# pkusys/Auncel

Hardware: AMD Instinct MI355X
Metric: queries/sec @ recall@10>=0.95, SIFT-10M d=128 IVF4096, 1/2/4/8 GPU (higher is better)
Workload: dtype u8

## Files before the change

auncel_amd/csrc/ivf_select.hip:

```cpp
#include "ivf_dev.h"

#include <algorithm>
#include <stdexcept>
#include <stdlib.h>
#include <string.h>
#include <string>
#include <type_traits>
#include <utility>

namespace amdivf {

struct RegHeap {
    uint32_t v0, v1;
    uint32_t s0, s1;
};

__device__ __forceinline__ void wl_u(uint32_t& reg, uint32_t val, int l) {
    uint32_t m0s;
    asm("s_mov_b32 %[m], m0\n\ts_mov_b32 m0, %[l]\n\ts_nop 0\n\tv_writelane_b32 %[r], %[v], m0\n\ts_mov_b32 m0, %[m]"
        : [r] "+v"(reg), [m] "=&s"(m0s)
        : [v] "s"(val), [l] "s"(l));
}

__device__ __forceinline__ void wl2_u(uint32_t& r0, uint32_t v0, uint32_t& r1, uint32_t v1, int l) {
// ... 382 lines not shown
        else high = middle - 1;
    }
    return (uint32_t)(low + 1);
}

constexpr uint32_t CURNUM_PAR_MAXK = 10;
template <bool IsMax>
__device__ inline uint32_t cur_num_par(const TraceLds& tr, const float* lut, const float* srt, const float* dwin, float* terms,
                                       uint32_t query_topk, int lane, uint32_t* err) {
    const int nterm = (int)query_topk * 15;
    unsigned long long errm = 0;
    for (int base = 0; base < nterm; base += 64) {
        const int idx = base + lane;
        uint32_t e = 0;
        if (idx < nterm) {
            const int m = idx / 15, i = idx - m * 15;
            uint32_t e0 = 0;
            const float kd = IsMax ? srt[m] : arcos_lut(lut, srt[m], &e0);
            const float b = dwin[i];
            float t = 0.f;
            if (!(b >= kd)) t = arcos_lut(lut, b / kd, &e);
            terms[idx] = t;
        }
        unsigned long long eb = __ballot(e != 0);
        while (eb) {
            const int l = __builtin_ctzll(eb);
            eb &= eb - 1;
            errm |= 1ull << ((base + l) / 15);
        }
    }
    wave_sync();
    float g = 0.f;
    if ((uint32_t)lane < query_topk) {
        float sum = 0.f;
#pragma unroll
        for (int i = 0; i < 15; i++) sum += terms[lane * 15 + i];
        g = trace_search(tr.x, tr.z, tr.n, sum);
    }
    const unsigned long long query_k = query_topk;
    const bool first_ok = (double)((float)query_k * g) <= (double)query_k * 1.005;
    const bool step_ok = (float)(lane + 1) * g <= (float)query_k;
    const unsigned long long mfirst = __ballot((uint32_t)lane == query_topk - 1 && first_ok);
    const unsigned long long mstep = __ballot((uint32_t)lane < query_topk && step_ok);
    wave_sync();
    unsigned long long high = query_k - 1, low = 0, middle = 0;
    if ((errm >> high) & 1) {
        *err = ERR_ARCOS_DOMAIN;
        return 0;
    }
    if (mfirst) return (uint32_t)query_k;
    while (low <= high) {
        middle = (low + high) / 2;
        if (middle <= 0) return 0;
        if ((errm >> middle) & 1) {
            *err = ERR_ARCOS_DOMAIN;
            return 0;
        }
        if ((mstep >> middle) & 1) low = middle + 1;
        else high = middle - 1;
    }
    return (uint32_t)(low + 1);
}

constexpr uint32_t SKEY_SENT = 0xff7fffffu;
constexpr uint32_t SPOS_NONE = 0xffffffffu;

struct SortedRegs {
    uint32_t k0, k1;
    uint32_t g0, g1;
};

__device__ __forceinline__ uint32_t wave_shr1(uint32_t x, uint32_t carry) {
    return (uint32_t)__builtin_amdgcn_update_dpp((int)carry, (int)x, 0x138 , 0xf, 0xf, false);
}

template <bool TWO> __device__ __forceinline__ uint32_t sr_key(const SortedRegs& r, int i) {
    if (!TWO) return rl_u(r.k0, i);
    const uint32_t a = rl_u(r.k0, i >> 1), b = rl_u(r.k1, i >> 1);
    return (i & 1) ? b : a;
}
template <bool TWO> __device__ __forceinline__ int sr_e0(int lane) { return TWO ? 2 * lane : lane; }
template <bool TWO> __device__ __forceinline__ int sr_e1(int lane) { return TWO ? 2 * lane + 1 : 128; }

template <bool TWO> __device__ __forceinline__ int sr_insert(SortedRegs& r, uint32_t key, uint32_t gpos, int lane) {
    (void)lane;
    const bool w0 = r.k0 > key;
    if (TWO) {
        const bool w1 = r.k1 > key;
        const int at = 128 - __builtin_popcountll(__ballot(w0)) - __builtin_popcountll(__ballot(w1));
        const uint32_t t0 = wave_shr1(r.k1, 0u), u0 = wave_shr1(r.g1, 0u);
        const bool p0 = t0 > key;
        const uint32_t n1k = w0 ? r.k0 : key, n1g = w0 ? r.g0 : gpos;
        r.k1 = w1 ? n1k : r.k1;
        r.g1 = w1 ? n1g : r.g1;
        r.k0 = w0 ? (p0 ? t0 : key) : r.k0;
        r.g0 = w0 ? (p0 ? u0 : gpos) : r.g0;
        return at;
    }
    const int at = 64 - __builtin_popcountll(__ballot(w0));
    const uint32_t t0 = wave_shr1(r.k0, 0u), u0 = wave_shr1(r.g0, 0u);
    const bool p0 = t0 > key;
    r.k0 = w0 ? (p0 ? t0 : key) : r.k0;
    r.g0 = w0 ? (p0 ? u0 : gpos) : r.g0;
    return at;
}

__device__ inline int64_t pair_of_gpos(const uint64_t* list_off, uint32_t nlist, uint32_t gpos) {
    uint32_t lo = 0, hi = nlist;
    while (hi - lo > 1) {
        const uint32_t mid = (lo + hi) >> 1;
        if (list_off[mid] <= gpos) lo = mid;
        else hi = mid;
    }
    return ((int64_t)lo << 32) | (int64_t)(gpos - list_off[lo]);
}

__host__ __device__ inline size_t replay_wave_bytes(int k, uint32_t nlist, bool geo, bool tune, bool train, uint32_t trace_cap) {
    (void)nlist;
    size_t b = (size_t)k * 16;
    if (geo) b += 16 * 4 + 16 * 4;
    if (tune) b += (size_t)trace_cap * 8;
    if (tune) b += CURNUM_PAR_MAXK * 15 * 4 + 8;
    if (train) b += (size_t)k * 4;
    return (b + 15) & ~(size_t)15;
}

template <bool IsMax, bool RH, int NLD, int KC>
__global__ __launch_bounds__(256) __attribute__((amdgpu_waves_per_eu(NLD == 16 ? 5 : 3))) void replay_kernel(ReplayArgs a) {
    extern __shared__ __align__(16) unsigned char smem[];
    const int lane = threadIdx.x & 63;
    const int wave = __builtin_amdgcn_readfirstlane(threadIdx.x >> 6);
    const bool tune = a.tuner.enabled != 0, training = a.train.enabled != 0, geo = tune || training;
    const int k = KC ? KC : a.k;
    const uint32_t nlist = a.nlist;
    const uint32_t max_num = nlist / 8 + 20;

    float* lut = reinterpret_cast<float*>(smem);
    if (geo) {
        const float* g = tune ? a.tuner.arcos : a.train.arcos;
        for (int i = threadIdx.x; i < 500; i += 256) lut[i] = g[i];
        __syncthreads();
    }
    const uint32_t li = blockIdx.x * 4 + wave;
    if (li >= (a.nq_dev ? *a.nq_dev : a.nq)) return;
    const uint32_t qi = a.qsel ? a.qsel[li] : li;
    if (a.done[qi]) return;

    unsigned char* base = smem + (geo ? 2000 : 0) + (size_t)wave * replay_wave_bytes(k, nlist, geo, tune, training, a.trace_cap);
    int64_t* href = reinterpret_cast<int64_t*>(base);
    float* hval = reinterpret_cast<float*>(base + (size_t)k * 8);
    float* srt = hval + k;
    float* dwin = srt + k;
    float* pend = dwin + (geo ? 16 : 0);
    float* trc = pend + (geo ? 16 : 0);
    float* terms = trc + (tune ? 2 * a.trace_cap : 0);
    float* gtrow = terms + (tune ? CURNUM_PAR_MAXK * 15 + 2 : 0);
    const float* gdtb = geo ? a.dtb + (size_t)qi * max_num : nullptr;

    for (int i = lane; i < k; i += 64) {
        hval[i] = a.heap_val[(size_t)qi * k + i];
        href[i] = a.heap_ref[(size_t)qi * k + i];
    }
    wave_sync();

    const unsigned long long id_q = a.id_offset + qi;
    const unsigned long long dbg_t0 = a.dbg ? __builtin_readcyclecounter() : 0;
    unsigned long long dbg_evals = 0, dbg_stream = 0, dbg_rule = 0, dbg_chunks = 0, dbg_probes = 0;
    uint32_t err = 0;
    uint32_t ik0 = a.stage[qi];
    const uint32_t loop_end = a.limit ? a.limit[qi] : a.total_nprobe;
    const uint32_t si = a.seg_by_slot ? qi : li;
    const uint32_t cnt = a.seg_count[si];
    const size_t seg0 = a.seg_begin ? (size_t)a.seg_begin[si] : (size_t)li * a.round_probes;
    unsigned long long nscan = a.nscan[qi];
    float pre_val = a.pre_val ? a.pre_val[qi] : 0.f;
    uint32_t stoped = a.stoped ? a.stoped[qi] : 0u;
    unsigned long long st_nlist = 0, st_nheap = 0, st_ndis = 0;

    constexpr bool VTWO = KC == 0 || KC > 63;
    auto stored = [](float x) { return IsMax ? fkey(x) : ~fkey(x); };
    auto unstored = [](uint32_t sk) { return fkey_inv(IsMax ? sk : ~sk); };
    VHeap vh{0u, 0u, 0u, 0u};
    const VHeapLane vc = vh_lane(lane);
    unsigned long long chain0 = 0, chain1 = 0;
    if (RH) {
        if (lane >= 1 && lane <= k) vh.k0 = stored(hval[lane - 1]);
        if (VTWO && lane + 64 <= k) vh.k1 = stored(hval[lane + 63]);
// ... 467 lines not shown
    const unsigned long long lt = (1ull << lane) - 1ull;
    for (uint32_t s0 = (blockIdx.x * 4u + (threadIdx.x >> 6)) * 8u; s0 < nseg; s0 += stride) {
        uint32_t m_n = 0;
        unsigned long long m_off = 0;
        if (lane < 8 && s0 + lane < nseg) {
            const int key = a.seg_list[s0 + lane];
            m_off = a.seg_off[s0 + lane];
            if (key >= 0 && (uint32_t)key < a.nlist) m_n = (uint32_t)(a.list_off[key + 1] - a.list_off[key]);
        }
        unsigned long long W[8];
#pragma unroll
        for (int r = 0; r < 8; r++) {
            const uint32_t n = rl_u(m_n, r);
            const unsigned long long off = ((unsigned long long)rl_u((uint32_t)(m_off >> 32), r) << 32) | rl_u((uint32_t)m_off, r);
            W[r] = (uint32_t)lane < ((n + 63u) >> 6) ? __builtin_nontemporal_load(a.mask + (off >> 6) + lane) : 0ull;
        }
#pragma unroll
        for (int r = 0; r < 8; r++) {
            if (s0 + r >= nseg) break;
            const uint32_t n = rl_u(m_n, r);
            const unsigned long long off = ((unsigned long long)rl_u((uint32_t)(m_off >> 32), r) << 32) | rl_u((uint32_t)m_off, r);
            const unsigned long long* mw = a.mask + (off >> 6) + lane;
            const float* row = a.dist + off + lane;
            const uint32_t words = (n + 63u) >> 6;
            uint32_t total = wave_sum_u32((uint32_t)__builtin_popcountll(W[r]));
            for (uint32_t b = 64; b < words; b += 64u)
                total += wave_sum_u32(b + lane < words ? (uint32_t)__builtin_popcountll(__builtin_nontemporal_load(mw + b)) : 0u);
            total = (uint32_t)__builtin_amdgcn_readfirstlane((int)total);
            uint2* ent = a.cl_ent + (size_t)(s0 + r) * CL_CAP;
            uint32_t report = total;
            if (total > CL_CAP) {
                uint32_t start = a.arena_per_xcd;
                if (lane == 0 && total <= a.arena_per_xcd &&
                    __hip_atomic_load(&a.cursor[32u * xcc_id()], __ATOMIC_RELAXED, __HIP_MEMORY_SCOPE_WORKGROUP) < a.arena_per_xcd)
                    start = xcd_local_add(&a.cursor[32u * xcc_id()], total);
                start = (uint32_t)__builtin_amdgcn_readfirstlane((int)start);
                if (start >= a.arena_per_xcd || total > a.arena_per_xcd - start) {
                    if (lane == 0) a.cl_cnt[s0 + r] = CL_WALK;
                    continue;
                }
                start += xcc_id() * a.arena_per_xcd;
                if (lane == 0) ent[0] = make_uint2(start, 0u);
                ent = a.arena + start;
            }
            uint32_t count = 0;
            auto put = [&](unsigned long long w, uint32_t b, int c, float x) {
                const unsigned long long bits = ((unsigned long long)rl_u((uint32_t)(w >> 32), c) << 32) | rl_u((uint32_t)w, c);
                const bool mine = (bits >> lane) & 1ull;
                const unsigned long long bal = __ballot(mine);
                if (mine) ent[count + (uint32_t)__builtin_popcountll(bal & lt)] = make_uint2((b + (uint32_t)c) * 64u + (uint32_t)lane, __float_as_uint(x));
                count += (uint32_t)__builtin_popcountll(bal);
            };
            for (uint32_t b = 0; b < words; b += 64u) {
                const unsigned long long w = b == 0 ? W[r] : (b + lane < words ? __builtin_nontemporal_load(mw + b) : 0ull);
                unsigned long long nz = __ballot(w != 0ull);
                while (nz) {
                    int c[4] = {-1, -1, -1, -1};
                    float x[4] = {0.f, 0.f, 0.f, 0.f};
#pragma unroll
                    for (int u = 0; u < 4; u++) {
                        if (nz) {
                            c[u] = __builtin_ctzll(nz);
                            nz &= nz - 1;
                            x[u] = __builtin_nontemporal_load(row + (size_t)(b + c[u]) * 64);
                        }
                    }
#pragma unroll
                    for (int u = 0; u < 4; u++)
                        if (c[u] >= 0) put(w, b, c[u], x[u]);
                }
            }
            if (lane == 0) a.cl_cnt[s0 + r] = report;
        }
    }
}

void launch_compact_rows(const CompactArgs& a, hipStream_t s) {
    const uint32_t want = a.nseg_dev ? a.nseg_hint : a.nseg;
    if (want == 0) return;
    const uint32_t grid = std::min<uint32_t>((want + 31u) / 32u, 8192u);
    LAUNCH(compact_rows_kernel, dim3(grid), dim3(256), 0, s, a);
}

template <bool IsMax, bool MASKED, bool TUNE, int KC>
__global__ __launch_bounds__(256) __attribute__((amdgpu_waves_per_eu(MASKED ? 4 : AUNCEL_SEL_WAVES))) void select_sorted_kernel(ReplayArgs a) {
    extern __shared__ __align__(16) unsigned char smem[];
    constexpr bool TWO = KC == 0 || KC > 64;
    const int lane = threadIdx.x & 63;
    const int wave = __builtin_amdgcn_readfirstlane(threadIdx.x >> 6);
    const int k = KC ? KC : a.k;
    const uint32_t nlist = a.nlist;
    const uint32_t max_num = nlist / 8 + 20;
    float* lut = reinterpret_cast<float*>(smem);
    if (TUNE) {
        for (int i = threadIdx.x; i < 500; i += 256) lut[i] = a.tuner.arcos[i];
        __syncthreads();
    }
    const uint32_t li = blockIdx.x * 4 + wave;
    if (li >= (a.nq_dev ? *a.nq_dev : a.nq)) return;
    const uint32_t qi = (uint32_t)__builtin_amdgcn_readfirstlane((int)(a.qsel ? a.qsel[li] : li));
    if (a.done[qi]) return;

    unsigned char* wbase = smem + (TUNE ? 2000 : 0) + (size_t)wave * select_wave_bytes(k, TUNE, !MASKED, a.trace_cap);
    uint32_t* mk = reinterpret_cast<uint32_t*>(wbase);
    uint32_t* mg = mk + 128;
    float* srt = reinterpret_cast<float*>(wbase + SEL_MERGE_BYTES);
    float* dwin = srt + k;
    float* trc = dwin + 16;
    float* terms = trc + (!MASKED && 2 * a.trace_cap < 640u ? 640u : 2 * a.trace_cap);
    uint32_t* fill = reinterpret_cast<uint32_t*>(TUNE ? reinterpret_cast<unsigned char*>(trc) : wbase + SEL_MERGE_BYTES);
    const float* gdtb = TUNE ? a.dtb + (size_t)qi * max_num : nullptr;

    SortedRegs sr{0xffffffffu, 0xffffffffu, SPOS_NONE, SPOS_NONE};
    const int e0 = sr_e0<TWO>(lane), e1 = sr_e1<TWO>(lane);
    if (e0 < k) {
        sr.k0 = okey<IsMax>(a.heap_val[(size_t)qi * k + e0]);
        sr.g0 = (uint32_t)a.heap_ref[(size_t)qi * k + e0];
    }
    if (TWO && e1 < k) {
        sr.k1 = okey<IsMax>(a.heap_val[(size_t)qi * k + e1]);
        sr.g1 = (uint32_t)a.heap_ref[(size_t)qi * k + e1];
    }
    uint32_t amb = (uint32_t)__builtin_amdgcn_readfirstlane((int)a.amb[qi]);
    uint32_t logn = (uint32_t)__builtin_amdgcn_readfirstlane((int)a.log_cnt[qi]);
    uint2* const qlog = a.log + (size_t)qi * a.log_cap;
    uint32_t log_v = 0, log_g = 0;
    if (!AUNCEL_SEL_BATCH && (uint32_t)lane < (logn & 63u)) {
        const uint2 e = qlog[(logn & ~63u) + lane];
        log_v = e.x;
        log_g = e.y;
    }
    auto worst_key = [&]() { return sr_key<TWO>(sr, k - 1); };
    uint32_t topk = worst_key();
    float top = okey_inv<IsMax>(topk);
    auto srt_from_regs = [&]() {
        if (e0 < k) srt[e0] = okey_inv<IsMax>(sr.k0);
        if (TWO && e1 < k) srt[e1] = okey_inv<IsMax>(sr.k1);
    };
    if (TUNE) {
        srt_from_regs();
        wave_sync();
    }

    const unsigned long long id_q = a.id_offset + qi;
    uint32_t err = 0;
    const uint32_t ik0 = (uint32_t)__builtin_amdgcn_readfirstlane((int)a.stage[qi]);
    const uint32_t loop_end = a.limit ? a.limit[qi] : a.total_nprobe;
    const uint32_t cnt = (uint32_t)__builtin_amdgcn_readfirstlane((int)a.seg_count[qi]);
    const size_t seg0 = (size_t)a.seg_begin[qi];
    unsigned long long nscan = a.nscan[qi];
    float pre_val = a.pre_val[qi];
    uint32_t stoped = a.stoped[qi];
    unsigned long long st_nlist = 0, st_ndis = 0;
    uint32_t st_nheap = 0;
    const unsigned long long dbg_t0 = a.dbg ? __builtin_readcyclecounter() : 0;
    unsigned long long dbg_rule = 0;
    uint32_t dbg_evals = 0, dbg_chunks = 0, dbg_walked = 0;

    uint32_t query_k = 0;
    float true_KD_K = 0.f, racc = 0.f;
    unsigned long long np = 0;
    int cached_ind = -1;
    bool have_pre = false, top_changed = true, srt_changed = true;
    uint32_t kept_pre = 0;
    TraceLds tr{trc, trc + a.trace_cap, 0};
    if (TUNE) {
        query_k = a.tuner.query_topk;
        if (a.tuner.gt_D) true_KD_K = a.tuner.gt_D[id_q * (unsigned long long)k + query_k - 1];
        racc = a.tuner.require_acc[id_q];
        np = a.tuner.my_nprobe[id_q];
    }
    const unsigned long long np_in = np;
    const uint32_t nl8 = nlist / 8;
    const bool overhead = TUNE && a.tuner.overhead != 0;
    const float mult = TUNE ? a.tuner.multipler : 1.f;
    const unsigned long long stops = (unsigned long long)(racc * 12);
    float kept_recall = 0.f;

    int ins_min = 128;
#if AUNCEL_SEL_BATCH
    uint32_t B_k = 0, B_g = 0;
    uint32_t bn = 0;
    auto flush = [&]() {
        if (bn == 0) return;
        const bool cand = (uint32_t)lane < bn;
        const uint32_t myk = cand ? B_k : 0xffffffffu;
        uint32_t pa = 0, w = 0, later = 0, sh0 = 0, sh1 = 0;
        for (uint32_t i = 0; i < bn; i++) {
            const uint32_t ki = rl_u(B_k, (int)i);
            uint32_t p = (uint32_t)__builtin_popcountll(__ballot(sr.k0 <= ki));
            if (TWO) p += (uint32_t)__builtin_popcountll(__ballot(sr.k1 <= ki));
            wl_u(pa, (uint32_t)__builtin_amdgcn_readfirstlane((int)p), __builtin_amdgcn_readfirstlane((int)i));
            w += (ki <= myk && (uint32_t)lane > i) ? 1u : 0u;
            later += (ki < myk && (uint32_t)lane < i) ? 1u : 0u;
            sh0 += ki < sr.k0 ? 1u : 0u;
            if (TWO) sh1 += ki < sr.k1 ? 1u : 0u;
        }
        const bool adm = cand && pa + w < (uint32_t)k;
        const unsigned long long am = __ballot(adm);
        const uint32_t nadm = (uint32_t)__builtin_popcountll(am);
        if (nadm) {
            const uint32_t rank = pa + w + later;
            const uint32_t r0 = (uint32_t)e0 + sh0, r1 = (uint32_t)e1 + sh1;
            wave_sync();
            if (e0 < k && r0 < (uint32_t)k) {
                mk[r0] = sr.k0;
                mg[r0] = sr.g0;
            }
            if (TWO && e1 < k && r1 < (uint32_t)k) {
                mk[r1] = sr.k1;
                mg[r1] = sr.g1;
            }
            if (adm && rank < (uint32_t)k) {
                mk[rank] = B_k;
                mg[rank] = B_g;
            }
            if (logn + nadm > a.log_cap) {
                err = ERR_LOG_OVERFLOW;
            } else if (adm) {
                const uint32_t at = logn + (uint32_t)__builtin_popcountll(am & ((1ull << lane) - 1ull));
                qlog[at] = make_uint2(__float_as_uint(okey_inv<IsMax>(B_k)), B_g);
            }
            logn += logn + nadm > a.log_cap ? 0u : nadm;
            st_nheap += nadm;
            const unsigned long long top_in = __ballot(adm && rank < query_k);
            if (top_in) ins_min = 0;
            wave_sync();
            const bool l0 = e0 < k, l1 = TWO && e1 < k;
            const uint32_t wk = mk[k - 1];
            const bool out0 = l0 && r0 >= (uint32_t)k && sr.k0 == wk, out1 = l1 && r1 >= (uint32_t)k && sr.k1 == wk;
            const bool outc = adm && rank >= (uint32_t)k && B_k == wk;
            if (l0) {
                sr.k0 = mk[e0];
                sr.g0 = mg[e0];
            }
            if (l1) {
                sr.k1 = mk[e1];
                sr.g1 = mg[e1];
            }
            if (wk != SKEY_SENT && __ballot(out0 || out1 || outc) != 0) amb = wk;
            topk = wk;
            top = okey_inv<IsMax>(wk);
        }
        bn = 0;
    };
    auto admit = [&](float val, uint32_t ckey, uint32_t gp) {
        (void)val;
        gp = (uint32_t)__builtin_amdgcn_readfirstlane((int)gp);
        wl2_u(B_k, (uint32_t)__builtin_amdgcn_readfirstlane((int)ckey), B_g, gp, __builtin_amdgcn_readfirstlane((int)bn));
        bn++;
        if (bn == 64u) flush();
    };
#else
    auto flush = [&]() {};
    auto admit = [&](float val, uint32_t ckey, uint32_t gp) {
        const uint32_t evicted = topk;
        gp = (uint32_t)__builtin_amdgcn_readfirstlane((int)gp);
        const int at = sr_insert<TWO>(sr, ckey, gp, lane);
        ins_min = at < ins_min ? at : ins_min;
        const uint32_t ln = (uint32_t)__builtin_amdgcn_readfirstlane((int)logn);
        if (ln >= a.log_cap) {
            err = ERR_LOG_OVERFLOW;
        } else {
            const bool me = (uint32_t)lane == (ln & 63u);
            log_v = me ? __float_as_uint(val) : log_v;
            log_g = me ? gp : log_g;
            if ((ln & 63u) == 63u) qlog[(ln & ~63u) + lane] = make_uint2(log_v, log_g);
            logn = ln + 1;
        }
        st_nheap++;
        const uint32_t wk = worst_key();
        if (wk == evicted && wk != SKEY_SENT) amb = wk;
        topk = wk;
        top = okey_inv<IsMax>(wk);
    };
#endif

    uint32_t win0 = 0;
    int m_key = -1;
    uint32_t m_n = 0, m_base = 0;
    const bool lists = MASKED && a.cl_cnt != nullptr;
    uint32_t m_cc = 0;
    uint2 E[8];
    auto load_window = [&](uint32_t w0) {
        win0 = w0;
        m_key = -1;
        m_n = 0;
        m_base = 0;
        const uint32_t pi = w0 + lane;
        if (lists) {
            m_cc = pi < cnt ? a.cl_cnt[seg0 + pi] : 0u;
            const uint2* ep = a.cl_ent + (seg0 + w0) * CL_CAP + lane;
#pragma unroll
            for (int j = 0; j < 8; j++) E[j] = w0 + 8u * j + ((uint32_t)lane >> 3) < cnt ? ep[64 * j] : make_uint2(0u, 0u);
        }
        if (pi < cnt) {
            m_key = a.seg_list[seg0 + pi];
            if (m_key >= 0 && (uint32_t)m_key < nlist) {
                const uint64_t o0 = a.list_off[m_key], o1 = a.list_off[m_key + 1];
                m_n = (uint32_t)(o1 - o0);
                m_base = a.identity_ids ? 0u : (uint32_t)o0;
            }
        }
    };
    load_window(0);
    unsigned long long region_off = cnt ? a.seg_off[seg0] : 0ull;
    region_off = ((unsigned long long)(uint32_t)__builtin_amdgcn_readfirstlane((int)(region_off >> 32)) << 32) |
                 (uint32_t)__builtin_amdgcn_readfirstlane((int)(uint32_t)region_off);

    const float* regionf = a.dist + region_off + lane;
    auto load_block = [&](const float* p) {
        f4 r;
        r.x = __builtin_nontemporal_load(p);
        r.y = __builtin_nontemporal_load(p + 64);
        r.z = __builtin_nontemporal_load(p + 128);
        r.w = __builtin_nontemporal_load(p + 192);
        return r;
    };
    f4 R0, R1, R2, R3;
    uint32_t gpos = 0;
    const unsigned long long* rmask = MASKED ? a.mask + (region_off >> 6) + lane : nullptr;
    const float* region1 = a.dist + region_off + lane;
    unsigned long long W = 0, Wn = 0;
    uint32_t wstep = 0;
    if (!MASKED) {
        R0 = load_block(regionf);
        R1 = load_block(regionf + 256);
        R2 = load_block(regionf + 512);
        R3 = load_block(regionf + 768);
    } else if (!lists) {
        W = __builtin_nontemporal_load(rmask);
        Wn = __builtin_nontemporal_load(rmask + 64);
    }
    uint32_t wpos = 0;

    auto dense_block = [&](const f4 x, uint32_t c0, uint32_t n, uint32_t lbase, uint32_t taken) {
        const uint32_t valid = n > c0 ? n - c0 : 0u;
        const uint32_t skip = taken > c0 ? taken - c0 : 0u;
        const uint32_t p0 = (uint32_t)lane, p1 = 64u + lane, p2 = 128u + lane, p3 = 192u + lane;
        const unsigned long long h0 = __ballot(hcmp<IsMax>(top, x.x) && p0 < valid && p0 >= skip);
        const unsigned long long h1 = __ballot(hcmp<IsMax>(top, x.y) && p1 < valid && p1 >= skip);
        const unsigned long long h2 = __ballot(hcmp<IsMax>(top, x.z) && p2 < valid && p2 >= skip);
        const unsigned long long h3 = __ballot(hcmp<IsMax>(top, x.w) && p3 < valid && p3 >= skip);
        auto walk = [&](unsigned long long h, const float xc, uint32_t g0) {
            while (h) {
                const int l = __builtin_ctzll(h);
                h &= h - 1;
                const float val = rl_f(xc, l);
                const uint32_t ck = okey<IsMax>(val);
                if (ck < topk) admit(val, ck, g0 + (uint32_t)l);
            }
        };
        const uint32_t g0 = lbase + c0;
        walk(h0, x.x, g0);
        walk(h1, x.y, g0 + 64u);
        walk(h2, x.z, g0 + 128u);
        walk(h3, x.w, g0 + 192u);
    };

    auto fill_first_k = [&](const f4 x, uint32_t n, uint32_t lbase) -> uint32_t {
        const uint32_t m = n < (uint32_t)k ? n : (uint32_t)k;
        uint32_t *fk = fill, *fv = fill + 128, *fg = fill + 256, *sk = fill + 384, *sg = fill + 512;
        const float xs[4] = {x.x, x.y, x.z, x.w};
        bool bad = false;
#pragma unroll
        for (int c = 0; c < 4; c++) bad = bad || (64u * c + lane < m && okey<IsMax>(xs[c]) >= SKEY_SENT);
        if (__ballot(bad) != 0) return 0u;
#pragma unroll
        for (int c = 0; c < 4; c++) {
            const uint32_t j = 64u * c + lane;
            if (j < m) {
                fk[j] = okey<IsMax>(xs[c]);
                fv[j] = __float_as_uint(xs[c]);
                fg[j] = lbase + j;
                qlog[j] = make_uint2(__float_as_uint(xs[c]), lbase + j);
            }
        }
        wave_sync();
        const uint32_t j0 = lane, j1 = lane + 64;
        const uint32_t k0v = j0 < m ? fk[j0] : 0u, k1v = j1 < m ? fk[j1] : 0u;
        uint32_t r0 = 0, r1 = 0;
        for (uint32_t i = 0; i < m; i++) {
            const uint32_t ki = fk[i];
            r0 += (ki < k0v || (ki == k0v && i < j0)) ? 1u : 0u;
            r1 += (ki < k1v || (ki == k1v && i < j1)) ? 1u : 0u;
        }
        if (j0 < m) {
            sk[r0] = k0v;
            sg[r0] = fg[j0];
        }
        if (j1 < m) {
            sk[r1] = k1v;
            sg[r1] = fg[j1];
        }
        wave_sync();
        if ((uint32_t)e0 < m) {
            sr.k0 = sk[e0];
            sr.g0 = sg[e0];
        }
        if (TWO && (uint32_t)e1 < m) {
            sr.k1 = sk[e1];
            sr.g1 = sg[e1];
        }
        logn = m;
        if ((uint32_t)lane < (m & 63u)) {
            log_v = fv[(m & ~63u) + lane];
            log_g = fg[(m & ~63u) + lane];
        }
        st_nheap += m;
        ins_min = 0;
        topk = worst_key();
        top = okey_inv<IsMax>(topk);
        wave_sync();
        return m;
    };
    bool fresh = !MASKED && logn == 0 && sr_key<TWO>(sr, 0) == SKEY_SENT;

    bool finished = false;
    uint32_t consumed = 0;
    for (uint32_t p = 0; p < cnt && !finished; p++) {
        const uint32_t ik = ik0 + p;
        consumed = p + 1;
        if (p >= win0 + 64) load_window(p);
        const int key = rl_i(m_key, (int)(p - win0));
        ins_min = 128;
        const uint32_t nheap0 = st_nheap;
        if (key >= 0) {
            if ((uint32_t)key >= nlist) {
                err = ERR_INVALID_KEY;
                finished = true;
                break;
            }
            const uint32_t n = rl_u(m_n, (int)(p - win0));
            if (n > 0) {
                st_nlist++;
                const uint32_t lbase = rl_u(m_base, (int)(p - win0));
                if (!MASKED) {
                    const uint32_t ngrp = (n + 1023u) >> 10;
                    uint32_t taken = 0;
                    if (fresh) {
                        taken = fill_first_k(R0, n, lbase);
                        fresh = false;
                    }
                    for (uint32_t g = 0; g < ngrp; g++) {
                        const float* nxt = regionf + (size_t)(gpos + 1) * 1024;
#define SEL_BLOCK(R, U)                                                                                                       \
    {                                                                                                                         \
        const f4 x = R;                                                                                                       \
        R = load_block(nxt + (U) * 256);                                                                                      \
        const float best = IsMax ? fminf(fminf(fminf(x.x, x.y), x.z), x.w) : fmaxf(fmaxf(fmaxf(x.x, x.y), x.z), x.w);         \
        if (__ballot(hcmp<IsMax>(top, best)) != 0) dense_block(x, g * 1024u + (U) * 256u, n, lbase, taken);                   \
    }
                        SEL_BLOCK(R0, 0)
                        SEL_BLOCK(R1, 1)
                        SEL_BLOCK(R2, 2)
                        SEL_BLOCK(R3, 3)
#undef SEL_BLOCK
                        gpos++;
                    }
                } else {
                    const uint32_t row_w0 = wpos, wend = wpos + ((n + 63u) >> 6);
                    if (lists) {
                        const int r = (int)(p - win0);
                        const uint32_t cc = rl_u(m_cc, r);
                        if (cc <= CL_CAP) {
                            if (cc) {
                                uint2 e = E[0];
#pragma unroll
                                for (int j = 1; j < 8; j++)
                                    if ((r >> 3) == j) e = E[j];
                                const int l0 = (r & 7) * 8;
                                for (uint32_t t = 0; t < cc; t++) {
                                    const float val = __uint_as_float(rl_u(e.y, l0 + (int)t));
                                    const uint32_t ck = okey<IsMax>(val);
                                    if (hcmp<IsMax>(top, val) && ck < topk) admit(val, ck, lbase + rl_u(e.x, l0 + (int)t));
                                }
                            }
                            wpos = wend;
                        } else if (cc != CL_WALK) {
                            uint2 e = E[0];
#pragma unroll
                            for (int j = 1; j < 8; j++)
                                if ((r >> 3) == j) e = E[j];
                            const uint2* al = a.cl_arena + rl_u(e.x, (r & 7) * 8) + lane;
                            for (uint32_t t0 = 0; t0 < cc; t0 += 64u) {
                                const bool in = t0 + (uint32_t)lane < cc;
                                const uint2 o = in ? al[t0] : make_uint2(0u, 0u);
                                unsigned long long m = __ballot(in && hcmp<IsMax>(top, __uint_as_float(o.y)));
                                while (m) {
                                    const int l = __builtin_ctzll(m);
                                    m &= m - 1;
                                    const float val = __uint_as_float(rl_u(o.y, l));
                                    const uint32_t ck = okey<IsMax>(val);
                                    if (ck < topk) admit(val, ck, lbase + rl_u(o.x, l));
                                }
                            }
                            wpos = wend;
                        } else {
                            if (a.dbg) dbg_walked++;
                            wstep = wpos >> 6;
                            W = __builtin_nontemporal_load(rmask + (size_t)wstep * 64);
                            Wn = __builtin_nontemporal_load(rmask + (size_t)(wstep + 1) * 64);
                        }
                    }
                    while (wpos < wend) {
                        const uint32_t s0 = wstep * 64u;
                        if (wpos >= s0 + 64u) {
                            W = Wn;
                            wstep++;
                            Wn = __builtin_nontemporal_load(rmask + (size_t)(wstep + 1) * 64);
                            continue;
                        }
                        const uint32_t lo = wpos - s0, hi = wend - s0 < 64u ? wend - s0 : 64u;
                        unsigned long long nz = __ballot(W != 0ull);
                        nz &= ~0ull << lo;
                        if (hi < 64u) nz &= (1ull << hi) - 1ull;
                        wpos = s0 + hi;
                        while (nz) {
                            int c0 = -1, c1 = -1, c2 = -1, c3 = -1;
                            float x0 = 0.f, x1 = 0.f, x2 = 0.f, x3 = 0.f;
                            c0 = __builtin_ctzll(nz);
                            nz &= nz - 1;
                            x0 = __builtin_nontemporal_load(region1 + (size_t)(s0 + c0) * 64);
                            if (nz) {
                                c1 = __builtin_ctzll(nz);
                                nz &= nz - 1;
                                x1 = __builtin_nontemporal_load(region1 + (size_t)(s0 + c1) * 64);
                            }
                            if (nz) {
                                c2 = __builtin_ctzll(nz);
                                nz &= nz - 1;
                                x2 = __builtin_nontemporal_load(region1 + (size_t)(s0 + c2) * 64);
                            }
                            if (nz) {
                                c3 = __builtin_ctzll(nz);
                                nz &= nz - 1;
                                x3 = __builtin_nontemporal_load(region1 + (size_t)(s0 + c3) * 64);
                            }
                            auto chunk = [&](int c, float x) {
                                if (c < 0) return;
                                if (a.dbg) dbg_chunks++;
                                const unsigned long long bits = ((unsigned long long)rl_u((uint32_t)(W >> 32), c) << 32) | rl_u((uint32_t)W, c);
                                const uint32_t cb = (s0 + (uint32_t)c - row_w0) * 64u;
                                unsigned long long m = __ballot(((bits >> lane) & 1) && hcmp<IsMax>(top, x));
                                while (m) {
                                    const int l = __builtin_ctzll(m);
                                    m &= m - 1;
                                    const float val = rl_f(x, l);
                                    const uint32_t ck = okey<IsMax>(val);
                                    if (ck < topk) admit(val, ck, lbase + cb + (uint32_t)l);
                                }
                            };
                            chunk(c0, x0);
                            chunk(c1, x1);
                            chunk(c2, x2);
                            chunk(c3, x3);
                        }
                    }
                    wpos = row_w0 + (((n + 1023u) >> 10) << 4);
                }
                nscan += n;
                st_ndis += n;
            }
        }
        flush();
        if (TUNE && st_nheap != nheap0) {
            wave_sync();
            srt_from_regs();
            wave_sync();
            srt_changed = true;
            if (ins_min < (int)query_k) top_changed = true;
        }
        if (a.max_codes && nscan >= a.max_codes) {
            finished = true;
            break;
        }
        if (loop_end && ik + 1 >= loop_end) finished = true;
        if (TUNE) {
            const unsigned long long dbg_r0 = a.dbg ? __builtin_readcyclecounter() : 0;
            const uint32_t stage = ik + 1;
            const bool fired = IsMax && np != 0 && !overhead;
            if (!fired) {
                const uint32_t tmp_stage = stage >= nl8 ? nl8 - 1 : stage;
                const uint32_t ind = tmp_stage <= 1u ? 0u : 32u - (uint32_t)__builtin_clz(tmp_stage - 1u);
                if ((int)ind != cached_ind) {
                    const uint32_t o = a.tuner.trace_off[ind], tn = a.tuner.trace_off[ind + 1] - o;
                    const float sc = a.tuner.std_m;
                    wave_sync();
                    for (uint32_t i = lane; i < tn; i += 64) {
                        trc[i] = a.tuner.trace_x[o + i];
                        trc[a.trace_cap + i] = a.tuner.trace_y[o + i] + sc * a.tuner.trace_std[o + i];
                    }
                    if (lane < 15) dwin[lane] = gdtb[(1u << ind) - 1 + lane];
                    tr.n = tn;
                    cached_ind = (int)ind;
                    have_pre = false;
                    wave_sync();
                }
                if (!IsMax && srt_changed) {
                    for (int i = lane; i < k; i += 64) (void)arcos_lut(lut, srt[i], &err);
                    err = wave_err(err);
                    if (err) {
                        finished = true;
                        break;
                    }
                }
                srt_changed = false;
                if (!have_pre || top_changed) {
                    dbg_evals++;
                    kept_pre = query_k <= CURNUM_PAR_MAXK ? cur_num_par<IsMax>(tr, lut, srt, dwin, terms, query_k, lane, &err)
                                                          : cur_num_lds<IsMax>(tr, lut, srt, dwin, query_k, lane, &err);
                    have_pre = true;
                    top_changed = false;
                    err = wave_err(err);
                    if (err) finished = true;
                    kept_recall = (float)kept_pre / (float)query_k;
                }
                float recall = kept_recall;
                const float max_val = IsMax ? fmaxf(-1.f, top) : fminf(FLT_MAX, top);
                if (stage > 1) {
                    if (max_val == pre_val) stoped++;
                    else stoped = 0;
                    if (stoped >= stops) recall = 1;
                }
                pre_val = max_val;
                if (!overhead) {
                    if (recall >= racc && np == 0) {
                        np = (unsigned long long)((float)stage * mult);
                        if (np >= nlist && lane == 0) a.tuner.t_recalls[id_q] = 1.f;
                    }
                    if (stage >= nl8 && np == 0) {
                        np = (unsigned long long)((float)stage * mult);
                        if (np >= nlist && lane == 0) a.tuner.t_recalls[id_q] = 1.f;
                    }
                }
            }
            if (overhead) {
                if (stage >= nl8) finished = true;
            } else if (np != 0 && np <= stage) {
                if (a.tuner.profile) {
                    uint32_t hits = 0;
                    for (int i = lane; i < k; i += 64) {
                        const float s = srt[i];
                        if (IsMax ? ((double)s <= (double)true_KD_K * 1.0005) : ((double)s >= (double)true_KD_K * 0.9995)) hits++;
                    }
                    for (int off = 32; off; off >>= 1) hits += __shfl_xor(hits, off);
                    if (lane == 0) a.tuner.t_recalls[id_q] = (float)hits / (float)query_k;
                }
                finished = true;
            }
            if (a.dbg) dbg_rule += __builtin_readcyclecounter() - dbg_r0;
        }
    }
    err = wave_err(err);

    if (lane == 0) {
        a.stage[qi] = ik0 + consumed;
        a.nscan[qi] = nscan;
        a.pre_val[qi] = pre_val;
        a.stoped[qi] = stoped;
        if (TUNE && np != np_in) a.tuner.my_nprobe[id_q] = np;
        if (a.qstat) {
            uint2 qs = a.qstat[qi];
            qs.x += (uint32_t)st_nlist;
            qs.y += (uint32_t)st_nheap;
            a.qstat[qi] = qs;
        }
        {
            unsigned long long* st = a.stats + 4 * xcc_id();
            if (st_nlist) xcd_local_add64(&st[0], st_nlist);
            if (st_ndis) xcd_local_add64(&st[1], st_ndis);
            if (st_nheap) xcd_local_add64(&st[2], (unsigned long long)st_nheap);
        }
        if (err) atomicMax(a.error, err);
        if (a.dbg) {
            a.dbg[(size_t)li * 8 + 0] = __builtin_readcyclecounter() - dbg_t0;
            a.dbg[(size_t)li * 8 + 1] = st_nheap;
            a.dbg[(size_t)li * 8 + 2] = st_ndis;
            a.dbg[(size_t)li * 8 + 3] = dbg_evals;
            a.dbg[(size_t)li * 8 + 4] = dbg_walked;
            a.dbg[(size_t)li * 8 + 5] = dbg_rule;
            a.dbg[(size_t)li * 8 + 6] = dbg_chunks;
            a.dbg[(size_t)li * 8 + 7] = consumed;
        }
        if (a.thr) a.thr[qi] = top;
        a.log_cnt[qi] = logn;
        a.log_snap[(size_t)(a.round & 1u) * a.nq_total + qi] = logn;
        if (finished || a.finalize_all || err) a.fin_round[qi] = a.round;
    }
    if (!AUNCEL_SEL_BATCH && (uint32_t)lane < (logn & 63u)) qlog[(logn & ~63u) + lane] = make_uint2(log_v, log_g);
    const bool in0 = e0 < k, in1 = TWO && e1 < k;
    if (finished || a.finalize_all || err) {
        const uint32_t p0 = wave_shr1(TWO ? sr.k1 : sr.k0, 0xfffffffeu), p1 = sr.k0;
        const bool dup = (in0 && lane >= 1 && sr.k0 == p0 && sr.k0 != SKEY_SENT) || (in1 && sr.k1 == p1 && sr.k1 != SKEY_SENT);
        const bool tainted = __ballot(dup) != 0 || worst_key() == amb;
        if (tainted && !err) {
            if (lane == 0) {
                a.tie_flag[qi] = 1;
                xcd_local_add64(&a.stats[4 * xcc_id() + 3], 1ull);
            }
        } else {
            auto put = [&](int i, uint32_t key, uint32_t g) {
                const bool empty = key == SKEY_SENT && g == SPOS_NONE;
                int64_t id = -1;
                if (!empty) id = a.identity_ids ? (int64_t)g : a.store_pairs ? pair_of_gpos(a.list_off, nlist, g) : a.ids[g];
                a.D[(size_t)qi * k + i] = empty ? hneutral<IsMax>() : okey_inv<IsMax>(key);
                a.I[(size_t)qi * k + i] = id;
            };
            if (in0) put(e0, sr.k0, sr.g0);
            if (in1) put(e1, sr.k1, sr.g1);
        }
        if (lane == 0) a.done[qi] = 1;
    } else {
        if (in0) {
            a.heap_val[(size_t)qi * k + e0] = okey_inv<IsMax>(sr.k0);
            a.heap_ref[(size_t)qi * k + e0] = sr.g0 == SPOS_NONE ? -1 : (int64_t)sr.g0;
        }
        if (in1) {
            a.heap_val[(size_t)qi * k + e1] = okey_inv<IsMax>(sr.k1);
            a.heap_ref[(size_t)qi * k + e1] = sr.g1 == SPOS_NONE ? -1 : (int64_t)sr.g1;
        }
        if (lane == 0) {
            a.amb[qi] = amb;
            if (a.unfinished) (void)xcd_local_add(&a.unfinished[xcc_id()], 1u);
        }
    }
}

void launch_select_sorted(const ReplayArgs& a, hipStream_t s) {
    if (a.nq == 0) return;
    const bool tune = a.tuner.enabled != 0;
    const size_t shmem = (tune ? 2000 : 0) + 4 * select_wave_bytes(a.k, tune, a.mask == nullptr, a.trace_cap);
    if (shmem > 160 * 1024) throw std::runtime_error("selection kernel: trace cache beyond LDS");
    const dim3 grid((a.nq + 3) / 4), block(256);
    auto go = [&](auto kern) {
        const hipError_t e = hipFuncSetAttribute(reinterpret_cast<const void*>(kern), hipFuncAttributeMaxDynamicSharedMemorySize, (int)shmem);
        if (e != hipSuccess) throw std::runtime_error(std::string("selection kernel: cannot reserve LDS: ") + hipGetErrorString(e));
        LAUNCH(kern, grid, block, shmem, s, a);
    };
    auto pick_k = [&](auto is_max, auto masked, auto tn) {
        constexpr bool M = decltype(is_max)::value, MK = decltype(masked)::value, T = decltype(tn)::value;
        if (a.k == 100) return go(select_sorted_kernel<M, MK, T, 100>);
        if (a.k == 10) return go(select_sorted_kernel<M, MK, T, 10>);
        return go(select_sorted_kernel<M, MK, T, 0>);
    };
    auto pick_t = [&](auto is_max, auto masked) {
        if (tune) pick_k(is_max, masked, std::true_type{});
        else pick_k(is_max, masked, std::false_type{});
    };
    auto pick_m = [&](auto is_max) {
        if (a.mask) pick_t(is_max, std::true_type{});
        else pick_t(is_max, std::false_type{});
    };
    if (a.metric == METRIC_L2) pick_m(std::true_type{});
    else pick_m(std::false_type{});
}

bool replay_sorted_applies(const ReplayArgs& a) {
    return a.log != nullptr && a.k >= 1 && a.k <= 128 && !a.train.enabled && !a.raw_heap_out;
}

void launch_replay(const ReplayArgs& a, hipStream_t s) {
    if (a.nq == 0) return;
    const bool tune = a.tuner.enabled != 0, train = a.train.enabled != 0, geo = tune || train;
    const size_t shmem = (geo ? 2000 : 0) + 4 * replay_wave_bytes(a.k, a.nlist, geo, tune, train, a.trace_cap);
    const dim3 grid((a.nq + 3) / 4), block(256);
    static const bool no_rh = getenv("AUNCEL_AMD_LDS_HEAP") != nullptr;
    if (replay_sorted_applies(a)) {
        launch_select_sorted(a, s);
        return;
    }
    const bool rh = a.k <= 127 && !no_rh;
    if (shmem > 160 * 1024)
        throw std::runtime_error("k = " + std::to_string(a.k) + " is beyond the selection kernel's LDS heap (" + std::to_string(shmem) +
                                 " bytes of 163840 per workgroup)");
    auto go = [&](auto kern) {
        const hipError_t e = hipFuncSetAttribute(reinterpret_cast<const void*>(kern), hipFuncAttributeMaxDynamicSharedMemorySize, (int)shmem);
        if (e != hipSuccess) throw std::runtime_error(std::string("selection kernel: cannot reserve LDS: ") + hipGetErrorString(e));
        LAUNCH(kern, grid, block, shmem, s, a);
    };
    const char* nld_s = getenv("AUNCEL_AMD_REPLAY_NLD");
    const int nld_env = nld_s ? atoi(nld_s) : 0;
    const bool wide = nld_env ? nld_env >= 32 : (a.nq_hint ? a.nq_hint : a.nq) <= 3072;
    auto pick = [&](auto is_max) {
        constexpr bool M = decltype(is_max)::value;
        if (!rh) return wide ? go(replay_kernel<M, false, 32, 0>) : go(replay_kernel<M, false, 16, 0>);
        if (a.k == 100) return wide ? go(replay_kernel<M, true, 32, 100>) : go(replay_kernel<M, true, 16, 100>);
        if (a.k == 10) return wide ? go(replay_kernel<M, true, 32, 10>) : go(replay_kernel<M, true, 16, 10>);
// ... 165 lines not shown
```

Before: 2.920 million.

## Drop payload tracking from sorted-register top-k insert and reconstruct positions at exit

In the non-batched, unmasked select path the sorted register heap now carries only keys during the scan. The per-insert payload shuffles and ballot popcounts are removed. The matching global positions are rebuilt once at the end by binary-searching the original heap entries and new log entries against the final sorted keys in LDS, with extra handling for duplicate keys. The tuning trigger now compares the minimum inserted key against the query_k-th key instead of tracking the insertion index, and the float threshold conversion is deferred to the end of each chunk. This cuts per-candidate VALU and cross-lane work but adds a reconstruction pass and extra LDS synchronisation, with a risk of mismatched ids when keys tie.

After: 2.889 million. 0.989x the previous value.

```diff
diff --git a/auncel_amd/csrc/ivf_select.hip b/auncel_amd/csrc/ivf_select.hip
--- a/auncel_amd/csrc/ivf_select.hip
+++ b/auncel_amd/csrc/ivf_select.hip
@@ -488,27 +488,30 @@
 template <bool TWO> __device__ __forceinline__ int sr_e0(int lane) { return TWO ? 2 * lane : lane; }
 template <bool TWO> __device__ __forceinline__ int sr_e1(int lane) { return TWO ? 2 * lane + 1 : 128; }
 
-template <bool TWO> __device__ __forceinline__ int sr_insert(SortedRegs& r, uint32_t key, uint32_t gpos, int lane) {
-    (void)lane;
+template <bool TWO, bool PAY> __device__ __forceinline__ void sr_insert(SortedRegs& r, uint32_t key, uint32_t gpos) {
     const bool w0 = r.k0 > key;
     if (TWO) {
         const bool w1 = r.k1 > key;
-        const int at = 128 - __builtin_popcountll(__ballot(w0)) - __builtin_popcountll(__ballot(w1));
-        const uint32_t t0 = wave_shr1(r.k1, 0u), u0 = wave_shr1(r.g1, 0u);
+        const uint32_t t0 = wave_shr1(r.k1, 0u);
         const bool p0 = t0 > key;
-        const uint32_t n1k = w0 ? r.k0 : key, n1g = w0 ? r.g0 : gpos;
+        if (PAY) {
+            const uint32_t u0 = wave_shr1(r.g1, 0u);
+            const uint32_t n1g = w0 ? r.g0 : gpos;
+            r.g1 = w1 ? n1g : r.g1;
+            r.g0 = w0 ? (p0 ? u0 : gpos) : r.g0;
+        }
+        const uint32_t n1k = w0 ? r.k0 : key;
         r.k1 = w1 ? n1k : r.k1;
-        r.g1 = w1 ? n1g : r.g1;
         r.k0 = w0 ? (p0 ? t0 : key) : r.k0;
+        return;
+    }
+    const uint32_t t0 = wave_shr1(r.k0, 0u);
+    const bool p0 = t0 > key;
+    if (PAY) {
+        const uint32_t u0 = wave_shr1(r.g0, 0u);
         r.g0 = w0 ? (p0 ? u0 : gpos) : r.g0;
-        return at;
-    }
-    const int at = 64 - __builtin_popcountll(__ballot(w0));
-    const uint32_t t0 = wave_shr1(r.k0, 0u), u0 = wave_shr1(r.g0, 0u);
-    const bool p0 = t0 > key;
+    }
     r.k0 = w0 ? (p0 ? t0 : key) : r.k0;
-    r.g0 = w0 ? (p0 ? u0 : gpos) : r.g0;
-    return at;
 }
 
 __device__ inline int64_t pair_of_gpos(const uint64_t* list_off, uint32_t nlist, uint32_t gpos) {
@@ -1142,6 +1145,8 @@
     LAUNCH(compact_rows_kernel, dim3(grid), dim3(256), 0, s, a);
 }
 
+__device__ __forceinline__ uint32_t wave_err_uni(uint32_t err) { return (uint32_t)__builtin_amdgcn_readfirstlane((int)wave_err(err)); }
+
 template <bool IsMax, bool MASKED, bool TUNE, int KC>
 __global__ __launch_bounds__(256) __attribute__((amdgpu_waves_per_eu(MASKED ? 4 : AUNCEL_SEL_WAVES))) void select_sorted_kernel(ReplayArgs a) {
     extern __shared__ __align__(16) unsigned char smem[];
@@ -1171,18 +1176,20 @@
     uint32_t* fill = reinterpret_cast<uint32_t*>(TUNE ? reinterpret_cast<unsigned char*>(trc) : wbase + SEL_MERGE_BYTES);
     const float* gdtb = TUNE ? a.dtb + (size_t)qi * max_num : nullptr;
 
+    constexpr bool PAY = MASKED || AUNCEL_SEL_BATCH;
     SortedRegs sr{0xffffffffu, 0xffffffffu, SPOS_NONE, SPOS_NONE};
     const int e0 = sr_e0<TWO>(lane), e1 = sr_e1<TWO>(lane);
     if (e0 < k) {
         sr.k0 = okey<IsMax>(a.heap_val[(size_t)qi * k + e0]);
-        sr.g0 = (uint32_t)a.heap_ref[(size_t)qi * k + e0];
+        if (PAY) sr.g0 = (uint32_t)a.heap_ref[(size_t)qi * k + e0];
     }
     if (TWO && e1 < k) {
         sr.k1 = okey<IsMax>(a.heap_val[(size_t)qi * k + e1]);
-        sr.g1 = (uint32_t)a.heap_ref[(size_t)qi * k + e1];
+        if (PAY) sr.g1 = (uint32_t)a.heap_ref[(size_t)qi * k + e1];
     }
     uint32_t amb = (uint32_t)__builtin_amdgcn_readfirstlane((int)a.amb[qi]);
     uint32_t logn = (uint32_t)__builtin_amdgcn_readfirstlane((int)a.log_cnt[qi]);
+    const uint32_t logn_in = logn;
     uint2* const qlog = a.log + (size_t)qi * a.log_cap;
     uint32_t log_v = 0, log_g = 0;
     if (!AUNCEL_SEL_BATCH && (uint32_t)lane < (logn & 63u)) {
@@ -1237,8 +1244,10 @@
     const unsigned long long stops = (unsigned long long)(racc * 12);
     float kept_recall = 0.f;
 
+    uint32_t ck_min = 0xffffffffu;
+    uint32_t kq = TUNE && query_k ? sr_key<TWO>(sr, (int)query_k - 1) : 0u;
+#if AUNCEL_SEL_BATCH
     int ins_min = 128;
-#if AUNCEL_SEL_BATCH
     uint32_t B_k = 0, B_g = 0;
     uint32_t bn = 0;
     auto flush = [&]() {
@@ -1314,10 +1323,10 @@
 #else
     auto flush = [&]() {};
     auto admit = [&](float val, uint32_t ckey, uint32_t gp) {
-        const uint32_t evicted = topk;
+        amb = topk;
         gp = (uint32_t)__builtin_amdgcn_readfirstlane((int)gp);
-        const int at = sr_insert<TWO>(sr, ckey, gp, lane);
-        ins_min = at < ins_min ? at : ins_min;
+        sr_insert<TWO, PAY>(sr, ckey, gp);
+        ck_min = ckey < ck_min ? ckey : ck_min;
         const uint32_t ln = (uint32_t)__builtin_amdgcn_readfirstlane((int)logn);
         if (ln >= a.log_cap) {
             err = ERR_LOG_OVERFLOW;
@@ -1329,10 +1338,8 @@
             logn = ln + 1;
         }
         st_nheap++;
-        const uint32_t wk = worst_key();
-        if (wk == evicted && wk != SKEY_SENT) amb = wk;
-        topk = wk;
-        top = okey_inv<IsMax>(wk);
+        topk = worst_key();
+        if (MASKED) top = okey_inv<IsMax>(topk);
     };
 #endif
 
@@ -1416,6 +1423,7 @@
         walk(h1, x.y, g0 + 64u);
         walk(h2, x.z, g0 + 128u);
         walk(h3, x.w, g0 + 192u);
+        top = okey_inv<IsMax>(topk);
     };
 
     auto fill_first_k = [&](const f4 x, uint32_t n, uint32_t lbase) -> uint32_t {
@@ -1447,20 +1455,20 @@
         }
         if (j0 < m) {
             sk[r0] = k0v;
-            sg[r0] = fg[j0];
+            if (PAY) sg[r0] = fg[j0];
         }
         if (j1 < m) {
             sk[r1] = k1v;
-            sg[r1] = fg[j1];
+            if (PAY) sg[r1] = fg[j1];
         }
         wave_sync();
         if ((uint32_t)e0 < m) {
             sr.k0 = sk[e0];
-            sr.g0 = sg[e0];
+            if (PAY) sr.g0 = sg[e0];
         }
         if (TWO && (uint32_t)e1 < m) {
             sr.k1 = sk[e1];
-            sr.g1 = sg[e1];
+            if (PAY) sr.g1 = sg[e1];
         }
         logn = m;
         if ((uint32_t)lane < (m & 63u)) {
@@ -1468,7 +1476,10 @@
             log_g = fg[(m & ~63u) + lane];
         }
         st_nheap += m;
+        ck_min = 0u;
+#if AUNCEL_SEL_BATCH
         ins_min = 0;
+#endif
         topk = worst_key();
         top = okey_inv<IsMax>(topk);
         wave_sync();
@@ -1483,7 +1494,10 @@
         consumed = p + 1;
         if (p >= win0 + 64) load_window(p);
         const int key = rl_i(m_key, (int)(p - win0));
+        ck_min = 0xffffffffu;
+#if AUNCEL_SEL_BATCH
         ins_min = 128;
+#endif
         const uint32_t nheap0 = st_nheap;
         if (key >= 0) {
             if ((uint32_t)key >= nlist) {
@@ -1629,7 +1643,13 @@
             srt_from_regs();
             wave_sync();
             srt_changed = true;
-            if (ins_min < (int)query_k) top_changed = true;
+#if AUNCEL_SEL_BATCH
+            if (ins_min < (int)query_k) ck_min = 0u;
+#endif
+            if (ck_min < kq) {
+                top_changed = true;
+                kq = sr_key<TWO>(sr, (int)query_k - 1);
+            }
         }
         if (a.max_codes && nscan >= a.max_codes) {
             finished = true;
@@ -1659,7 +1679,7 @@
                 }
                 if (!IsMax && srt_changed) {
                     for (int i = lane; i < k; i += 64) (void)arcos_lut(lut, srt[i], &err);
-                    err = wave_err(err);
+                    err = wave_err_uni(err);
                     if (err) {
                         finished = true;
                         break;
@@ -1670,9 +1690,10 @@
                     dbg_evals++;
                     kept_pre = query_k <= CURNUM_PAR_MAXK ? cur_num_par<IsMax>(tr, lut, srt, dwin, terms, query_k, lane, &err)
                                                           : cur_num_lds<IsMax>(tr, lut, srt, dwin, query_k, lane, &err);
+                    kept_pre = (uint32_t)__builtin_amdgcn_readfirstlane((int)kept_pre);
                     have_pre = true;
                     top_changed = false;
-                    err = wave_err(err);
+                    err = wave_err_uni(err);
                     if (err) finished = true;
                     kept_recall = (float)kept_pre / (float)query_k;
                 }
@@ -1712,7 +1733,7 @@
             if (a.dbg) dbg_rule += __builtin_readcyclecounter() - dbg_r0;
         }
     }
-    err = wave_err(err);
+    err = wave_err_uni(err);
 
     if (lane == 0) {
         a.stage[qi] = ik0 + consumed;
@@ -1750,10 +1771,77 @@
     }
     if (!AUNCEL_SEL_BATCH && (uint32_t)lane < (logn & 63u)) qlog[(logn & ~63u) + lane] = make_uint2(log_v, log_g);
     const bool in0 = e0 < k, in1 = TWO && e1 < k;
+    if (!PAY) {
+        uint32_t *fk = fill, *fp = fill + 128, *fc = fill + 256, *ft = fill + 384;
+        wave_sync();
+        fk[e0] = in0 ? sr.k0 : 0xffffffffu;
+        fp[e0] = SPOS_NONE;
+        fc[e0] = 0u;
+        if (TWO) {
+            fk[e1] = in1 ? sr.k1 : 0xffffffffu;
+            fp[e1] = SPOS_NONE;
+            fc[e1] = 0u;
+        } else {
+            fk[64 + lane] = 0xffffffffu;
+            fp[64 + lane] = SPOS_NONE;
+            fc[64 + lane] = 0u;
+        }
+        wave_sync();
+        auto place = [&](uint32_t key, uint32_t g, bool valid) {
+            if (__ballot(valid && key <= topk) == 0) return;
+            uint32_t s = 0;
+#pragma unroll
+            for (uint32_t step = 64; step; step >>= 1) s += fk[s + step - 1] < key ? step : 0u;
+            const bool hit = valid && fk[s] == key;
+            const bool run = hit && s < 127u && fk[s + 1] == key;
+            if (hit) ft[s] = (uint32_t)lane;
+            wave_sync();
+            const bool clash = hit && ft[s] != (uint32_t)lane;
+            unsigned long long todo = __ballot(hit);
+            if (__ballot(run || clash) == 0) {
+                if (hit && fc[s] == 0u) {
+                    fp[s] = g;
+                    fc[s] = 1u;
+                }
+                todo = 0;
+            }
+            while (todo) {
+                const int l = __builtin_ctzll(todo);
+                todo &= todo - 1;
+                const uint32_t s1 = rl_u(s, l), x1 = rl_u(key, l), g1 = rl_u(g, l);
+                wave_sync();
+                const uint32_t at = s1 + (uint32_t)__builtin_amdgcn_readfirstlane((int)fc[s1]);
+                wave_sync();
+                if (lane == 0 && at < 128u && fk[at] == x1) {
+                    fp[at] = g1;
+                    fc[s1] = at - s1 + 1u;
+                }
+            }
+            wave_sync();
+        };
+        for (int i = lane; i < (TWO ? 128 : 64); i += 64) {
+            const bool in = i < k;
+            const uint32_t ck = in ? okey<IsMax>(a.heap_val[(size_t)qi * k + i]) : SKEY_SENT;
+            const uint32_t g = in ? (uint32_t)a.heap_ref[(size_t)qi * k + i] : SPOS_NONE;
+            place(ck, g, ck != SKEY_SENT);
+        }
+        for (uint32_t b = logn_in & ~63u; b < logn; b += 64u) {
+            const uint32_t i = b + (uint32_t)lane;
+            uint32_t v = log_v, g = log_g;
+            if (b != (logn & ~63u)) {
+                const uint2 e = qlog[i];
+                v = e.x;
+                g = e.y;
+            }
+            place(okey<IsMax>(__uint_as_float(v)), g, i >= logn_in && i < logn);
+        }
+        sr.g0 = fp[e0];
+        if (TWO) sr.g1 = fp[e1];
+    }
     if (finished || a.finalize_all || err) {
         const uint32_t p0 = wave_shr1(TWO ? sr.k1 : sr.k0, 0xfffffffeu), p1 = sr.k0;
         const bool dup = (in0 && lane >= 1 && sr.k0 == p0 && sr.k0 != SKEY_SENT) || (in1 && sr.k1 == p1 && sr.k1 != SKEY_SENT);
-        const bool tainted = __ballot(dup) != 0 || worst_key() == amb;
+        const bool tainted = __ballot(dup) != 0 || (topk == amb && topk != SKEY_SENT);
         if (tainted && !err) {
             if (lane == 0) {
                 a.tie_flag[qi] = 1;
@@ -1763,7 +1851,7 @@
             auto put = [&](int i, uint32_t key, uint32_t g) {
                 const bool empty = key == SKEY_SENT && g == SPOS_NONE;
                 int64_t id = -1;
-                if (!empty) id = a.identity_ids ? (int64_t)g : a.store_pairs ? pair_of_gpos(a.list_off, nlist, g) : a.ids[g];
+                if (!empty && (PAY || g != SPOS_NONE)) id = a.identity_ids ? (int64_t)g : a.store_pairs ? pair_of_gpos(a.list_off, nlist, g) : a.ids[g];
                 a.D[(size_t)qi * k + i] = empty ? hneutral<IsMax>() : okey_inv<IsMax>(key);
                 a.I[(size_t)qi * k + i] = id;
             };
```
